# yechuan51/huffman

Hardware: AMD Instinct MI355X
Metric: encode + decode throughput GB/s and % HBM3E peak, 16 GiB Zipf(1.1), 1/2/4/8 GPU (higher is better)
Workload: dtype u8; 1 GPU; 16 GiB Zipf(1.1) bytes per GPU: hist16 -> codebook -> pack -> decode, one global bit stream; bytes_per_gpu=17179869184, total_bytes=17179869184, symbols_per_gpu=8589934592, parallelism=single, payload_bytes_rank0=12416072164, max_code_len=22

## Files before the change

### huffman_amd/csrc/hz_kernels.hip

```cpp
#include <stdio.h>
#include <stdlib.h>

#include <type_traits>

#include "hz_device.h"

namespace hz {

struct DecArgs {
    const uint32_t* words;
    uint64_t nwords;
    uint32_t bit_adj;
    uint64_t nsym;
    uint64_t nblocks;
    const unsigned long long* starts;
    const unsigned long long* subs;
    uint64_t start0;
    const uint32_t* lds_img;
    uint32_t lds_words;
    uint32_t region_words;
    int k;
    int min_len;
    int max_len;
    int level_bits;
// ... 362 lines not shown
                }
                x = make_uint4(q[0], q[1], q[2], q[3]);
            }
            if (DESC)
                reinterpret_cast<uint4*>(stg)[npc_max - 1 - p] = make_uint4(bswap32(x.w), bswap32(x.z), bswap32(x.y), bswap32(x.x));
            else
                reinterpret_cast<uint4*>(stg)[p] = make_uint4(bswap32(x.x), bswap32(x.y), bswap32(x.z), bswap32(x.w));
        }
    }
    for (uint32_t p = (uint32_t)lane + kStageUnroll * kWave; p < npc; p += kWave) {
        const uint4 x = dec_stage_load(a, w0 + 4ull * p);
        if (DESC)
            reinterpret_cast<uint4*>(stg)[npc_max - 1 - p] = make_uint4(bswap32(x.w), bswap32(x.z), bswap32(x.y), bswap32(x.x));
        else
            reinterpret_cast<uint4*>(stg)[p] = make_uint4(bswap32(x.x), bswap32(x.y), bswap32(x.z), bswap32(x.w));
    }
}

constexpr int kPfStep = 4;
template <typename A>
HZ_DEV void dec_wave_pipe(const A& a, const uint32_t* lds, uint32_t* stg, uint32_t slot, uint64_t b,
                          uint64_t stride, int lane) {
    const uint32_t* l2g = a.l2;
    constexpr int C = kChainsPerLane;
    static_assert(C == 4, "two halves of two chains");
    PipeMeta mc, mn, mn2;
    uint4 sc[kStageUnroll], sn[kStageUnroll];
    dec_meta_load(a, b, lane, mc);
    dec_meta_load(a, b + stride, lane, mn);
    dec_stage_prefetch(a, mc, lane, sc);
    for (; b < a.nblocks; b += stride) {
        uint64_t w0;
        dec_stage_commit(a, mc, slot >> 2, stg, lane, sc, w0);
        uint32_t off[C];
        dec_chain_offsets(mc.sub, mc.b0, mc.b1 - mc.b0, lane, off);
        const uint32_t base = (uint32_t)(mc.b0 + a.bit_adj - (w0 << 5));
        uint32_t pos[C];
#pragma unroll
        for (int c = 0; c < C; ++c) pos[c] = base + off[c];
        __builtin_amdgcn_wave_barrier();
        uint32_t pk[kSPT / 2];
        PipeLane st[C];
        uint32_t g[C];
        auto finish = [&](int c, int q) {
            const uint32_t ee = (st[c].e >> 31) ? st[c].e : g[c];
            pos[c] += lut_leaf_len(ee);
            const uint32_t sym = lut_leaf_sym(ee);
            const int i = (c * kChainSyms + q) >> 1;
            if (q & 1) pk[i] |= sym << 16;
            else pk[i] = sym;
        };
        auto issue2 = [&](int c) {
            dec_pipe_lds2(a, lds, stg, pos[c], pos[c + 1], st[c], st[c + 1]);
            g[c] = l2g[st[c].gi];
            g[c + 1] = l2g[st[c + 1].gi];
        };
        issue2(0);
#pragma unroll
        for (int q = 0; q < kChainSyms; ++q) {
            issue2(2);
            if (q == kPfStep) {
                dec_stage_prefetch(a, mn, lane, sn);
                dec_meta_load(a, b + 2 * stride, lane, mn2);
            }
            finish(0, q);
            finish(1, q);
            if (q + 1 < kChainSyms) issue2(0);
            finish(2, q);
            finish(3, q);
        }
        __builtin_amdgcn_wave_barrier();
        dec_store(a, b, lane, pk);
        mc = mn;
        mn = mn2;
#pragma unroll
        for (int u = 0; u < kStageUnroll; ++u) sc[u] = sn[u];
    }
}

template <typename A>
HZ_DEV void dec_wave_pipe2(const A& a, const uint32_t* lds, uint32_t* stg, uint32_t slot, uint64_t b,
                           uint64_t stride, int lane) {
    constexpr int C = 2 * kChainsPerLane;
    static_assert(kChainsPerLane == 4, "four pairs of chains over two blocks");
    const __amdgpu_buffer_rsrc_t l2r = lut_l2_rsrc(a.l2);
    [[maybe_unused]] const uint32_t stg_bit = (uint32_t)(stg - lds) * 32u - 1u;
    PipeMeta mc[2], mn[2], mn2[2];
    uint4 sc[2][kStageUnroll], sn[2][kStageUnroll];
#pragma unroll
    for (int j = 0; j < 2; ++j) {
        dec_meta_load(a, b + j, lane, mc[j]);
        dec_meta_load(a, b + stride + j, lane, mn[j]);
    }
#pragma unroll
    for (int j = 0; j < 2; ++j) dec_stage_prefetch(a, mc[j], lane, sc[j]);
    for (; b < a.nblocks; b += stride) {
        uint32_t p1[C];
#pragma unroll
        for (int j = 0; j < 2; ++j) {
            uint64_t w0;
            dec_stage_commit<true>(a, mc[j], slot >> 2, stg + j * slot, lane, sc[j], w0);
            uint32_t off[kChainsPerLane];
            dec_chain_offsets(mc[j].sub, mc[j].b0, mc[j].b1 - mc[j].b0, lane, off);
            const uint32_t top = (uint32_t)(stg - lds) + (uint32_t)(j + 1) * slot - 1u;
            const uint32_t base = top * 32u - (uint32_t)(mc[j].b0 + a.bit_adj - (w0 << 5));
#pragma unroll
            for (int c = 0; c < kChainsPerLane; ++c) p1[j * kChainsPerLane + c] = base - off[c];
        }
        __builtin_amdgcn_wave_barrier();
        uint32_t pk[2][kSPT / 2];
        PipeLane st[C];
        uint32_t g[C];
        auto finish = [&](int c, int q) {
            const uint32_t ee = st[c].e > g[c] ? st[c].e : g[c];
            p1[c] -= ee >> 24;
            const int i = ((c % kChainsPerLane) * kChainSyms + q) >> 1;
            if (q & 1) pk[c / kChainsPerLane][i] = __builtin_amdgcn_perm(ee, pk[c / kChainsPerLane][i], 0x06050201u);
            else pk[c / kChainsPerLane][i] = ee;
        };
        auto issue4 = [&](int c, int q) {
            __builtin_amdgcn_s_setprio(2);
            dec_pipe_ldsn<4>(a, lds, p1 + c, st + c, 16u * (uint32_t)q);
#pragma unroll
            for (int t = 0; t < 4; ++t)
                g[c + t] = __builtin_amdgcn_raw_buffer_load_b32(l2r, st[c + t].gi, 0, 0);
            __builtin_amdgcn_s_setprio(0);
        };
        issue4(0, 0);
#pragma unroll
        for (int q = 0; q < kChainSyms; ++q) {
            issue4(4, q);
            if (q == kPfStep) {
#pragma unroll
                for (int j = 0; j < 2; ++j) dec_stage_prefetch(a, mn[j], lane, sn[j]);
#pragma unroll
                for (int j = 0; j < 2; ++j) dec_meta_load(a, b + 2 * stride + j, lane, mn2[j]);
            }
#pragma unroll
            for (int c = 0; c < 4; ++c) finish(c, q);
            if (q + 1 < kChainSyms) issue4(0, q + 1);
#pragma unroll
            for (int c = 4; c < 8; ++c) finish(c, q);
        }
        __builtin_amdgcn_wave_barrier();
#pragma unroll
        for (int j = 0; j < 2; ++j)
            if (b + j < a.nblocks) dec_store(a, b + j, lane, pk[j]);
#pragma unroll
        for (int j = 0; j < 2; ++j) {
            mc[j] = mn[j];
            mn[j] = mn2[j];
#pragma unroll
            for (int u = 0; u < kStageUnroll; ++u) sc[j][u] = sn[j][u];
        }
    }
}

constexpr int kDecPipe2Threads = 512;
template <int MODE, bool WIDE, int PIPE>
__global__ __launch_bounds__(PIPE == 2 ? kDecPipe2Threads : 1024) void k_decode(DecArgs a) {
    extern __shared__ __attribute__((aligned(16))) uint32_t lds[];
    copy_lds_table(lds, a.lds_img, a.lds_words);
    const int lane = threadIdx.x & 63;
    const uint32_t wid = wave_id();
    const uint32_t slot = (uint32_t)__builtin_amdgcn_readfirstlane((int)dec_slot_words(a.starts[a.nblocks + 1], a.max_len));
    const uint32_t nwave = blockDim.x >> 6;
    if constexpr (PIPE == 2) {
        uint32_t nw2 = a.region_words / (2 * slot);
        nw2 = nw2 < nwave ? nw2 : nwave;
        if (nw2 > 0) {
            if (wid >= nw2) return;
            const uint64_t b = 2 * ((uint64_t)blockIdx.x * nw2 + wid), stride = 2 * (uint64_t)gridDim.x * nw2;
            dec_wave_pipe2(a, lds, lds + a.lds_words + wid * 2 * slot, slot, b, stride, lane);
            return;
        }
    }
    uint32_t nw = a.region_words / slot;
    nw = nw < nwave ? nw : nwave;
    if (wid >= nw) return;
    uint32_t* stg = lds + a.lds_words + wid * slot;
    const uint64_t b = (uint64_t)blockIdx.x * nw + wid, stride = (uint64_t)gridDim.x * nw;
    if constexpr (PIPE != 0) {
        dec_wave_pipe(a, lds, stg, slot, b, stride, lane);
    } else {
        for (uint64_t bb = b; bb < a.nblocks; bb += stride) dec_group<MODE, WIDE, 1>(a, lds, stg, slot, bb, lane);
    }
}

HZ_DEV void fixed16_step(const uint16_t* t16, const uint32_t (&ww)[5], uint32_t pos, uint32_t (&o)[4]) {
    const uint32_t sh = pos & 31;
#pragma unroll
    for (int t = 0; t < 4; ++t) {
        const uint32_t cw = sh ? __builtin_amdgcn_alignbit(ww[t], ww[t + 1], 32u - sh) : ww[t];
        o[t] = (uint32_t)t16[cw >> 16] | ((uint32_t)t16[cw & 0xffffu] << 16);
    }
}

__global__ __launch_bounds__(1024) void k_decode_fixed16_blk(DecArgs a, uint64_t nb) {
    extern __shared__ __attribute__((aligned(16))) uint32_t lds[];
    copy_lds_table(lds, a.lds_img, a.lds_words);
    const uint16_t* t16 = reinterpret_cast<const uint16_t*>(lds);
    const uint64_t p0 = (a.starts ? a.starts[0] : a.start0) + a.bit_adj;
    const uint32_t* w = a.words + (p0 >> 5);
    const u32x4a4* w4 = reinterpret_cast<const u32x4a4*>(w);
    uint4* o4 = reinterpret_cast<uint4*>(a.out);
    const int lane = threadIdx.x & 63;
    const uint64_t W = (uint64_t)gridDim.x * (blockDim.x >> 6);
    uint64_t b = (uint64_t)blockIdx.x * (blockDim.x >> 6) + (threadIdx.x >> 6);
    constexpr uint32_t kBW = kBlockSyms / 2;
    auto load = [&](uint64_t bb, u32x4a4 (&x)[kChainsPerLane], uint32_t& nw) {
        bb = bb < nb ? bb : 0;
#pragma unroll
        for (int c = 0; c < kChainsPerLane; ++c) x[c] = w4[bb * (kBW / 4) + c * kWave + lane];
        nw = w[(bb + 1) * kBW];
    };
    u32x4a4 nx[kChainsPerLane];
    uint32_t nn = 0;
    if (b < nb) load(b, nx, nn);
    for (; b < nb; b += W) {
        u32x4a4 x[kChainsPerLane];
#pragma unroll
        for (int c = 0; c < kChainsPerLane; ++c) x[c] = nx[c];
        const uint32_t after = nn;
        load(b + W, nx, nn);
#pragma unroll
        for (int c = 0; c < kChainsPerLane; ++c) {
            uint32_t nxt = (uint32_t)__builtin_amdgcn_update_dpp(0, (int)x[c].x, kDppWaveShl1, 0xf, 0xf, false);
            const uint32_t first_next = c + 1 < kChainsPerLane ? readlane(x[c + 1 < kChainsPerLane ? c + 1 : c].x, 0) : after;
            if (lane == 63) nxt = first_next;
            const uint32_t ww[5] = {bswap32(x[c].x), bswap32(x[c].y), bswap32(x[c].z), bswap32(x[c].w), bswap32(nxt)};
            uint32_t o[4];
            fixed16_step(t16, ww, (uint32_t)p0, o);
            store_nt16(o4 + b * (kBlockSyms / 8) + c * kWave + lane, make_uint4(o[0], o[1], o[2], o[3]));
        }
    }
}

// ... 2228 lines not shown
```

### huffman_amd/csrc/hz_pack.hip

```cpp
#include <mutex>
#include <set>
#include <utility>

#include "hz_device.h"

namespace hz {

hipError_t ensure_lds_limit(const void* fn, int bytes) {
    int dev = 0;
    hipError_t e = hipGetDevice(&dev);
    if (e != hipSuccess) return e;
    static std::mutex mu;
    static std::set<std::pair<std::pair<const void*, int>, int>> done;
    std::lock_guard<std::mutex> lk(mu);
    const auto key = std::make_pair(std::make_pair(fn, dev), bytes);
    if (done.count(key)) return hipSuccess;
    if ((e = hipFuncSetAttribute(fn, hipFuncAttributeMaxDynamicSharedMemorySize, bytes)) != hipSuccess) return e;
    done.insert(key);
    return hipSuccess;
}

struct PackArgs {
    const uint8_t* in;
    uint64_t nsym;
    uint64_t nblocks;
    const uint32_t* lds_img;
    uint32_t lds_words;
    const unsigned long long* wide;
    const uint32_t* esc;
    const uint32_t* len8_img;
    uint32_t hot_mask;
    uint32_t hw_mask;
    uint32_t* out;
    uint64_t out_words;
    uint32_t lead;
    unsigned long long* blk;
    const unsigned long long* blk_start;
    unsigned long long* index;
    unsigned long long* index_sub;
    uint32_t* err;
    uint32_t slot_words;
    const unsigned long long* rstart;
    uint64_t bpr, nranges;
    unsigned long long* cold;
};

template <int MODE> struct PackEnt { using T = uint32_t; static constexpr int kShift = 26; };
template <> struct PackEnt<ENC_WIDE> { using T = uint64_t; static constexpr int kShift = 56; };
template <int MODE>
HZ_DEV uint32_t ent_len(typename PackEnt<MODE>::T e) {
    if constexpr (MODE == ENC_WIDE) return (uint32_t)(e >> 56);
    else return __builtin_amdgcn_ubfe((uint32_t)e, 26, 5);
}

template <typename T, int SH>
HZ_DEV T pack_dense_one(const uint32_t* lds, uint32_t s) {
    const uint32_t bit = s * 17u;
    const uint32_t w = bit >> 5;
    const uint64_t two = ((uint64_t)lds[w + 1] << 32) | lds[w];
    const uint32_t f = (uint32_t)(two >> (bit & 31)) & 0x1ffffu;
    const uint32_t L = f ? 16u - (uint32_t)__builtin_ctz(f) : 0u;
    return f ? (T)((L << SH) | (f >> (17u - L))) : (T)0;
}

struct PackIn {
    uint32_t raw[kSPT / 2];
    uint32_t psym;
    uint64_t bstart;
};

HZ_DEV void pack_prefetch(const PackArgs& a, uint64_t blk, int lane, PackIn& x) {
    const uint64_t sym0 = blk * kBlockSyms + (uint64_t)lane * kSPT;
    const uint64_t ls = sym0 + kSPT <= a.nsym ? sym0 : 0;
    const uint4* p = reinterpret_cast<const uint4*>(a.in + 2 * ls);
#pragma unroll
    for (int q = 0; q < kSPT / 8; ++q) {
        const uint4 v = p[q];
        x.raw[4 * q] = v.x; x.raw[4 * q + 1] = v.y; x.raw[4 * q + 2] = v.z; x.raw[4 * q + 3] = v.w;
    }
    const uint64_t ps = blk ? blk * kBlockSyms - 32 + (uint64_t)(lane & 31) : 0;
    x.psym = *reinterpret_cast<const uint16_t*>(a.in + 2 * ps);
    x.bstart = a.blk_start ? a.blk_start[blk] : 0;
}

struct HotLook {
    uint32_t x[kSPT], mk[kSPT], v[kSPT];
    uint32_t xx, xmk, xv;
};
template <bool FULL>
HZ_DEV void hot_issue(const PackArgs& a, const uint32_t (&raw)[kSPT / 2], uint32_t xs, HotLook& h, int nvalid = kSPT) {
    const uint32_t m2 = a.hot_mask | (a.hot_mask << 16);
    uint32_t ad[kSPT];
#pragma unroll
    for (int j = 0; j < kSPT / 2; ++j) {
        const uint32_t r = raw[j];
        const uint32_t sgn = __builtin_bit_cast(uint32_t, __builtin_bit_cast(hz_i16x2, r) >> (hz_i16x2){15, 15});
        const uint32_t sl = r ^ (sgn & m2);
        const uint32_t hi8 = __builtin_bit_cast(uint32_t, __builtin_bit_cast(hz_u16x2, sl) >> (hz_u16x2){8, 8});
        uint32_t hw, a0, a1;
        asm("v_bitop3_b32 %0, %1, %2, %3 bitop3:0x6c" : "=v"(hw) : "s"(a.hw_mask), "v"(sl), "v"(hi8));
        asm("v_lshlrev_b32_sdwa %0, %1, %2 dst_sel:DWORD dst_unused:UNUSED_PAD src0_sel:DWORD src1_sel:WORD_0"
            : "=v"(a0) : "v"(2u), "v"(hw));
        asm("v_lshlrev_b32_sdwa %0, %1, %2 dst_sel:DWORD dst_unused:UNUSED_PAD src0_sel:DWORD src1_sel:WORD_1"
            : "=v"(a1) : "v"(2u), "v"(hw));
        ad[2 * j] = a0;
        ad[2 * j + 1] = a1;
    }
#pragma unroll
    for (int k = 0; k < kSPT; ++k) {
        h.x[k] = lds_at(ad[k]);
        if (!FULL) h.x[k] = k < nvalid ? h.x[k] : 0u;
    }
    uint32_t xslot = xs ^ ((uint32_t)((int32_t)(xs << 16) >> 31) & a.hot_mask);
    xslot = hot_word(xslot & 0x7fffu) << 2;
    h.xx = lds_at(xslot);
    const char* esc = reinterpret_cast<const char*>(a.esc);
#pragma unroll
    for (int k = 0; k < kSPT; ++k) {
        const uint32_t tag = (k & 1) ? raw[k >> 1] : raw[k >> 1] << 16;
        h.mk[k] = (uint32_t)((int32_t)(h.x[k] ^ tag) >> 31);
        h.v[k] = *reinterpret_cast<const uint32_t*>(esc + (ad[k] & h.mk[k]));
    }
    h.xmk = (uint32_t)((int32_t)(h.xx ^ (xs << 16)) >> 31);
    h.xv = *reinterpret_cast<const uint32_t*>(esc + (xslot & h.xmk));
}
HZ_DEV void hot_finish(const HotLook& h, uint32_t (&e)[kSPT], uint32_t& xe) {
#pragma unroll
    for (int k = 0; k < kSPT; ++k) {
        uint32_t r;
        asm volatile("v_bfi_b32 %0, %1, %2, %3" : "=v"(r) : "v"(h.mk[k]), "v"(h.v[k]), "v"(h.x[k]));
        e[k] = r;
    }
    uint32_t r;
    asm volatile("v_bfi_b32 %0, %1, %2, %3" : "=v"(r) : "v"(h.xmk), "v"(h.xv), "v"(h.xx));
    xe = r;
}

struct NoMid {
    HZ_DEV void operator()() const {}
};
template <int MODE, bool FULL, typename Mid = NoMid>
HZ_DEV void pack_lookup(const PackArgs& a, const uint32_t* lds, uint64_t sym0, int nvalid, uint32_t (&raw)[kSPT / 2],
                        typename PackEnt<MODE>::T (&e)[kSPT], uint32_t xs, typename PackEnt<MODE>::T& xe,
                        Mid mid = Mid()) {
    using T = typename PackEnt<MODE>::T;
    constexpr int SH = PackEnt<MODE>::kShift;
    if (!FULL) {
#pragma unroll
        for (int k = 0; k < kSPT / 2; ++k) {
            uint32_t w = 0;
            if (2 * k < nvalid) w = (uint32_t)a.in[2 * (sym0 + 2 * k)] | ((uint32_t)a.in[2 * (sym0 + 2 * k) + 1] << 8);
            if (2 * k + 1 < nvalid)
                w |= ((uint32_t)a.in[2 * (sym0 + 2 * k + 1)] | ((uint32_t)a.in[2 * (sym0 + 2 * k + 1) + 1] << 8)) << 16;
            raw[k] = w;
        }
    }
    if constexpr (MODE == ENC_DENSE) {
#pragma unroll
        for (int k = 0; k < kSPT; ++k) {
            const uint32_t s = (raw[k >> 1] >> (16 * (k & 1))) & 0xffffu;
            const uint32_t bit = s * 17u;
            const uint32_t w = bit >> 5;
            const uint64_t two = ((uint64_t)lds[w + 1] << 32) | lds[w];
            const uint32_t f = (uint32_t)(two >> (bit & 31)) & 0x1ffffu;
            const uint32_t L = f ? 16u - (uint32_t)__builtin_ctz(f) : 0u;
            e[k] = ((FULL || k < nvalid) && f) ? (T)((L << SH) | (f >> (17u - L))) : (T)0;
        }
        xe = pack_dense_one<T, SH>(lds, xs);
        mid();
    } else if constexpr (MODE == ENC_HOT) {
        HotLook h;
        hot_issue<FULL>(a, raw, xs, h, nvalid);
        mid();
        hot_finish(h, e, xe);
    } else {
#pragma unroll
        for (int k = 0; k < kSPT; ++k) {
            const uint32_t s = (raw[k >> 1] >> (16 * (k & 1))) & 0xffffu;
            e[k] = (FULL || k < nvalid) ? (T)a.wide[s] : (T)0;
        }
        xe = (T)a.wide[xs];
        mid();
    }
}

constexpr int kCountThreads = 1024;
constexpr int kCountUnroll = 2;

__global__ __launch_bounds__(kCountThreads) void k_pack_count(PackArgs a) {
    extern __shared__ __attribute__((aligned(16))) uint32_t lds[];
    {
        const uint4* src = reinterpret_cast<const uint4*>(a.len8_img);
        uint4* dst = reinterpret_cast<uint4*>(lds);
        for (uint32_t i = threadIdx.x; i < kLen8LdsBytes / 16; i += blockDim.x) dst[i] = src[i];
        __syncthreads();
    }
    const uint8_t* l8 = reinterpret_cast<const uint8_t*>(lds);
    const int lane = threadIdx.x & 63;
    const uint64_t W = (uint64_t)gridDim.x * (blockDim.x >> 6);
    const uint64_t full = a.nsym / kBlockSyms;
    uint64_t blk = (uint64_t)blockIdx.x * (blockDim.x >> 6) + (threadIdx.x >> 6);
    for (; blk + (kCountUnroll - 1) * W < full; blk += kCountUnroll * W) {
        uint4 v[kCountUnroll][kSPT / 8];
#pragma unroll
        for (int u = 0; u < kCountUnroll; ++u) {
            const uint4* p = reinterpret_cast<const uint4*>(a.in + 2 * (blk + u * W) * kBlockSyms) + lane;
#pragma unroll
            for (int q = 0; q < kSPT / 8; ++q) v[u][q] = p[q * kWave];
        }
#pragma unroll
        for (int u = 0; u < kCountUnroll; ++u) {
            uint32_t n = 0;
#pragma unroll
            for (int q = 0; q < kSPT / 8; ++q) {
                const uint32_t wd[4] = {v[u][q].x, v[u][q].y, v[u][q].z, v[u][q].w};
#pragma unroll
                for (int k = 0; k < 8; ++k) n += l8[len8_index((wd[k >> 1] >> (16 * (k & 1))) & 0xffffu)];
            }
// ... 68 lines not shown
    }
}

constexpr int kPackMaxWaves = 8;
constexpr double kPackSlotMargin = 1.12;
constexpr int kPackWriteThreads = 64 * kPackMaxWaves;
constexpr int kPackCopyIters = 16;

template <int MODE>
struct PackBlk {
    typename PackEnt<MODE>::T e[kSPT];
    typename PackEnt<MODE>::T pe;
    uint32_t n, ex_n, bits;
    uint32_t nc[kChainsPerLane];
    int nvalid;
};

template <int MODE, bool FULL_ONLY = false, typename Mid = NoMid>
HZ_DEV void pack_block_lookup(const PackArgs& a, const uint32_t* lds, uint64_t blk, int lane, PackIn& in,
                              PackBlk<MODE>& b, Mid mid = Mid()) {
    const uint64_t sym0 = blk * kBlockSyms + (uint64_t)lane * kSPT;
    if constexpr (FULL_ONLY) {
        b.nvalid = kSPT;
        pack_lookup<MODE, true>(a, lds, sym0, b.nvalid, in.raw, b.e, in.psym, b.pe, mid);
        return;
    }
    b.nvalid = sym0 >= a.nsym ? 0 : (a.nsym - sym0 >= (uint64_t)kSPT ? kSPT : (int)(a.nsym - sym0));
    if (__ballot(b.nvalid != kSPT) == 0)
        pack_lookup<MODE, true>(a, lds, sym0, b.nvalid, in.raw, b.e, in.psym, b.pe, mid);
    else
        pack_lookup<MODE, false>(a, lds, sym0, b.nvalid, in.raw, b.e, in.psym, b.pe, mid);
}

struct PackOut {
    bool pending, fits;
    uint64_t base4, blk, bstart, sub;
    uint32_t sh4, nwords;
};

HZ_DEV void pack_copyout(const PackArgs& a, const uint32_t* slot, int lane, const PackOut& p) {
    if (!p.pending) return;
    if (p.fits) {
        const uint32_t sh4 = p.sh4;
        const uint32_t wend = sh4 + p.nwords;
        const uint32_t cf = sh4 ? 1u : 0u, cl = wend >> 2;
        const uint32_t nhead = sh4 ? 4u - sh4 : 0u, ntail = wend & 3u;
        {
            const uint32_t i = (uint32_t)lane < nhead ? sh4 + (uint32_t)lane : sh4;
            a.out[p.base4 + i] = bswap32(slot[i]);
        }
#pragma unroll
        for (int it = 0; it < kPackCopyIters / 4; ++it) {
            uint32_t c = cf + (uint32_t)lane + (uint32_t)it * kWave;
            c = c < cl ? c : cl - 1;
            const uint4 v = reinterpret_cast<const uint4*>(slot)[c];
            reinterpret_cast<uint4*>(a.out + p.base4)[c] = make_uint4(bswap32(v.x), bswap32(v.y), bswap32(v.z), bswap32(v.w));
        }
        {
            const uint32_t i = (uint32_t)lane < ntail ? 4u * cl + (uint32_t)lane : sh4;
            a.out[p.base4 + i] = bswap32(slot[i]);
        }
    }
    if (a.index) {
        a.index_sub[p.blk * kWave + lane] = p.sub;
        if (lane == 0) a.index[p.blk] = p.bstart;
    }
    __builtin_amdgcn_wave_barrier();
}

template <int MODE>
HZ_DEV void pack_block_count(int lane, PackBlk<MODE>& b) {
    uint32_t n = 0;
#pragma unroll
    for (int k = 0; k < kSPT; ++k) {
        if (k % kChainSyms == 0) b.nc[k / kChainSyms] = n;
        n += ent_len<MODE>(b.e[k]);
    }
    const uint32_t sn = wave_incl_sum(n);
    b.n = n;
    b.ex_n = sn - n;
    b.bits = readlane(sn, 63);
}

template <int MODE, bool SLOT_ONLY = false>
HZ_DEV void pack_block_emit(const PackArgs& a, uint32_t* slot, uint64_t blk, int lane, const PackBlk<MODE>& b,
                            uint64_t bstart, uint64_t& max_bits, PackOut* defer = nullptr) {
    using T = typename PackEnt<MODE>::T;
    constexpr int SH = PackEnt<MODE>::kShift;
    constexpr T CMASK = (T(1) << SH) - 1;
    const uint64_t sym0 = blk * kBlockSyms + (uint64_t)lane * kSPT;
    const uint32_t n = b.n, ex_n = b.ex_n;
    const uint64_t bend = bstart + b.bits;
    uint32_t ptail = a.lead;
    if (blk > 0) {
        uint32_t pn = ent_len<MODE>(b.pe);
        uint32_t pt = (uint32_t)(b.pe & CMASK);
        auto step = [&](uint32_t on, uint32_t ot) {
            pt = pn >= 32 ? pt : ((ot << pn) | pt);
            pn += on;
        };
        step(dpp0<kDppRowShr1>(pn), dpp0<kDppRowShr1>(pt));
        step(dpp0<kDppRowShr2>(pn), dpp0<kDppRowShr2>(pt));
        step(dpp0<kDppRowShr4>(pn), dpp0<kDppRowShr4>(pt));
        step(dpp0<kDppRowShr8>(pn), dpp0<kDppRowShr8>(pt));
        step(dpp0<kDppRowBcast15, 0xa>(pn), dpp0<kDppRowBcast15, 0xa>(pt));
        ptail = readlane(pt, 31);
    }
    const uint64_t o = bstart + ex_n;
    const bool fits = ((bend + 31) >> 5) <= a.out_words;
    if (!fits && lane == 0) atomicOr(a.err, 4u);
    const bool last = blk + 1 == a.nblocks;
    const uint64_t wfirst = bstart >> 5;
    const uint32_t nwords = (uint32_t)((bend >> 5) - wfirst);
    const uint32_t sh4 = (uint32_t)(wfirst & 3);
    if (SLOT_ONLY || (slot && !last && nwords + sh4 <= a.slot_words)) {
        uint32_t* sl = slot + sh4;
        uint64_t acc = 0;
        if constexpr (MODE == ENC_WIDE) {
            uint32_t na = (uint32_t)(o & 31);
            pack_emit<MODE, true>(b.e, acc, na, sl + (uint32_t)((o >> 5) - wfirst), true);
        } else {
            pack_emit_lds<MODE>(b.e, acc, (uint32_t)(o - (wfirst << 5)), sl);
        }
        const uint32_t prev = (uint32_t)__builtin_amdgcn_update_dpp((int)ptail, (int)(uint32_t)acc, kDppWaveShr1,
                                                                    0xf, 0xf, false);
        const uint32_t h = (uint32_t)(o & 31);
        if (h) sl[(uint32_t)((o >> 5) - wfirst)] |= prev << (32 - h);
        __builtin_amdgcn_wave_barrier();
        if (MODE != ENC_WIDE && defer) {
            defer->pending = true;
            defer->fits = fits;
            defer->base4 = wfirst & ~3ull;
            defer->sh4 = sh4;
            defer->nwords = nwords;
            defer->blk = blk;
            defer->bstart = bstart;
            uint64_t sub = 0;
#pragma unroll
            for (int c = 0; c < kChainsPerLane; ++c)
                sub |= (uint64_t)(((uint32_t)bstart + ex_n + b.nc[c]) & 0xffffu) << (16 * c);
            defer->sub = sub;
            max_bits = b.bits > max_bits ? b.bits : max_bits;
            return;
        }
        if (fits) {
            if constexpr (MODE != ENC_WIDE) {
                const uint64_t base4 = wfirst & ~3ull;
                const uint32_t wend = sh4 + nwords;
                const uint32_t cf = sh4 ? 1u : 0u, cl = wend >> 2;
                const uint32_t nhead = sh4 ? 4u - sh4 : 0u, ntail = wend & 3u;
                {
                    const uint32_t i = (uint32_t)lane < nhead ? sh4 + (uint32_t)lane : sh4;
                    a.out[base4 + i] = bswap32(slot[i]);
                }
#pragma unroll
                for (int it = 0; it < kPackCopyIters / 4; ++it) {
                    uint32_t c = cf + (uint32_t)lane + (uint32_t)it * kWave;
                    c = c < cl ? c : cl - 1;
                    const uint4 v = reinterpret_cast<const uint4*>(slot)[c];
                    reinterpret_cast<uint4*>(a.out + base4)[c] =
                        make_uint4(bswap32(v.x), bswap32(v.y), bswap32(v.z), bswap32(v.w));
                }
                {
                    const uint32_t i = (uint32_t)lane < ntail ? 4u * cl + (uint32_t)lane : sh4;
                    a.out[base4 + i] = bswap32(slot[i]);
                }
            } else {
                for (uint32_t w = lane; w < nwords; w += kWave) a.out[wfirst + w] = bswap32(sl[w]);
            }
        }
        __builtin_amdgcn_wave_barrier();
    } else if constexpr (!SLOT_ONLY) {
        uint64_t t64 = 0;
#pragma unroll
        for (int k = 0; k < kSPT; ++k) {
            const uint32_t L = ent_len<MODE>(b.e[k]);
            t64 = L ? ((t64 << L) | (uint64_t)(b.e[k] & CMASK)) : t64;
        }
        uint32_t tn = n, st = (uint32_t)t64;
#pragma unroll
        for (int d = 1; d < 64; d <<= 1) {
            const uint32_t on = shfl_up_u32(tn, d), ot = shfl_up_u32(st, d);
            if (lane >= d) {
                st = tn >= 32 ? st : (tn == 0 ? ot : ((ot << tn) | st));
                tn += on;
            }
        }
        uint32_t ex_t = shfl_up_u32(st, 1);
        if (lane == 0) ex_t = 0;
        const uint32_t pre = ex_n >= 32 ? ex_t : (ex_n == 0 ? ptail : ((ptail << ex_n) | ex_t));
        uint32_t na = (uint32_t)(o & 31);
        uint64_t acc = na ? (uint64_t)(pre & ((1u << na) - 1u)) : 0ull;
        uint32_t* dst = a.out + (o >> 5);
        pack_emit<MODE, false>(b.e, acc, na, dst, fits);
        dst += (uint32_t)(((o & 31) + n) >> 5);
        if (fits && b.nvalid > 0 && sym0 + (uint64_t)b.nvalid == a.nsym && na > 0)
            *dst = bswap32((uint32_t)(acc << (32 - na)));
    }
    if (a.index) {
        uint64_t sub = 0;
#pragma unroll
        for (int c = 0; c < kChainsPerLane; ++c)
            sub |= (uint64_t)(((uint32_t)bstart + ex_n + b.nc[c]) & 0xffffu) << (16 * c);
        a.index_sub[blk * kWave + lane] = sub;
        if (lane == 0) {
            a.index[blk] = bstart;
            if (last) a.index[a.nblocks] = bend;
        }
        max_bits = bend - bstart > max_bits ? bend - bstart : max_bits;
    }
}


template <int MODE, bool RNG, bool SPLIT>
__global__ __launch_bounds__(kPackWriteThreads) void k_pack_write(PackArgs a) {
    extern __shared__ __attribute__((aligned(16))) uint32_t lds[];
    if constexpr (MODE != ENC_WIDE) copy_lds_table(lds, a.lds_img, a.lds_words);
    const int lane = threadIdx.x & 63;
    constexpr bool kSplit = SPLIT && MODE != ENC_WIDE;
    uint32_t* slot = a.slot_words ? lds + a.lds_words + (threadIdx.x >> 6) * a.slot_words : nullptr;
    const uint64_t W = (uint64_t)gridDim.x * (blockDim.x >> 6);
    const uint64_t gw = (uint64_t)blockIdx.x * (blockDim.x >> 6) + (threadIdx.x >> 6);
    uint64_t max_bits = 0;
    uint64_t blk = gw, r = gw, rend = 0, run = 0;
    if (RNG) {
        blk = r < a.nranges ? r * a.bpr : a.nblocks;
        rend = blk + a.bpr < a.nblocks ? blk + a.bpr : a.nblocks;
        run = r < a.nranges ? a.rstart[r] : 0;
    }
    PackOut po;
    po.pending = false;
    if constexpr (MODE == ENC_HOT && kSplit) {
        auto next = [&](uint64_t b, bool& newr, uint64_t& nrun) -> uint64_t {
            newr = false;
            nrun = 0;
            if (!RNG) return b + W;
            if (b + 1 < rend) return b + 1;
            r += W;
            newr = true;
            const uint64_t n = r < a.nranges ? r * a.bpr : a.nblocks;
            rend = n + a.bpr < a.nblocks ? n + a.bpr : a.nblocks;
            nrun = r < a.nranges ? a.rstart[r] : 0;
            return n;
        };
        bool nb_newr;
        uint64_t nb_run;
        uint64_t nb = next(blk, nb_newr, nb_run);
        PackIn nx;
        HotLook hl;
        uint64_t bst_cur = run;
        if (blk < a.nblocks) {
            PackIn cur;
            pack_prefetch(a, blk, lane, cur);
            hot_issue<true>(a, cur.raw, cur.psym, hl);
            if (!RNG) bst_cur = cur.bstart;
            pack_prefetch(a, nb < a.nblocks ? nb : blk, lane, nx);
        }
        while (blk < a.nblocks) {
            bool nn_newr;
            uint64_t nn_run;
            const uint64_t nnb = next(nb, nn_newr, nn_run);
            PackBlk<MODE> b;
            hot_finish(hl, b.e, b.pe);
            b.nvalid = kSPT;
            __builtin_amdgcn_s_setprio(2);
            hot_issue<true>(a, nx.raw, nx.psym, hl);
            __builtin_amdgcn_s_setprio(0);
            const uint64_t nbst = nx.bstart;
            pack_copyout(a, slot, lane, po);
            po.pending = false;
            const uint64_t pb = nnb < a.nblocks ? nnb : (nb < a.nblocks ? nb : blk);
            pack_prefetch(a, pb, lane, nx);
            pack_block_count<MODE>(lane, b);
            const uint64_t bst = bst_cur;
            const uint64_t wfirst = bst >> 5;
            const uint32_t nwords = (uint32_t)(((bst + b.bits) >> 5) - wfirst), sh4 = (uint32_t)(wfirst & 3);
            if (blk + 1 == a.nblocks || nwords + sh4 > a.slot_words) {
                if (lane == 0) {
                    const unsigned long long i = atomicAdd(a.cold, 1ull);
                    a.cold[1 + 2 * i] = blk;
                    a.cold[2 + 2 * i] = bst;
                }
            } else {
                pack_block_emit<MODE, true>(a, slot, blk, lane, b, bst, max_bits, &po);
            }
            if (RNG) run = nb_newr ? nb_run : run + b.bits;
            bst_cur = RNG ? run : nbst;
            blk = nb;
            nb = nnb;
            nb_newr = nn_newr;
            nb_run = nn_run;
        }
        pack_copyout(a, slot, lane, po);
        if (a.index && lane == 0 && max_bits) atomicMax(a.index + a.nblocks + 1, (unsigned long long)max_bits);
        return;
    }
    PackIn nx;
    if (blk < a.nblocks) pack_prefetch(a, blk, lane, nx);
    while (blk < a.nblocks) {
        uint64_t nb = blk + W, nrun = 0;
        bool newr = false;
        if (RNG) {
            if (blk + 1 < rend) {
                nb = blk + 1;
            } else {
                r += W;
                newr = true;
                nb = r < a.nranges ? r * a.bpr : a.nblocks;
                rend = nb + a.bpr < a.nblocks ? nb + a.bpr : a.nblocks;
                nrun = r < a.nranges ? a.rstart[r] : 0;
            }
        }
        PackIn cur = nx;
        PackBlk<MODE> b;
        pack_block_lookup<MODE, kSplit>(a, lds, blk, lane, cur, b, [&]() { pack_copyout(a, slot, lane, po); });
        po.pending = false;
        pack_prefetch(a, nb < a.nblocks ? nb : blk, lane, nx);
        pack_block_count<MODE>(lane, b);
        const uint64_t bst = RNG ? run : cur.bstart;
        if constexpr (kSplit) {
            const uint64_t wfirst = bst >> 5;
            const uint32_t nwords = (uint32_t)(((bst + b.bits) >> 5) - wfirst), sh4 = (uint32_t)(wfirst & 3);
            if (blk + 1 == a.nblocks || nwords + sh4 > a.slot_words) {
                if (lane == 0) {
                    const unsigned long long i = atomicAdd(a.cold, 1ull);
                    a.cold[1 + 2 * i] = blk;
                    a.cold[2 + 2 * i] = bst;
                }
            } else {
                pack_block_emit<MODE, true>(a, slot, blk, lane, b, bst, max_bits, &po);
            }
        } else {
            pack_block_emit<MODE>(a, slot, blk, lane, b, bst, max_bits, &po);
        }
        if (RNG) run = newr ? nrun : run + b.bits;
        blk = nb;
    }
    pack_copyout(a, slot, lane, po);
    if (a.index && lane == 0 && max_bits) atomicMax(a.index + a.nblocks + 1, (unsigned long long)max_bits);
}

template <int MODE>
__global__ __launch_bounds__(kPackWriteThreads) void k_pack_cold(PackArgs a) {
    extern __shared__ __attribute__((aligned(16))) uint32_t lds[];
    const uint64_t n = a.cold[0];
    const uint64_t waves = blockDim.x >> 6, W = (uint64_t)gridDim.x * waves;
    if ((uint64_t)blockIdx.x * waves >= n) return;
    if constexpr (MODE != ENC_WIDE) copy_lds_table(lds, a.lds_img, a.lds_words);
    const int lane = threadIdx.x & 63;
    uint64_t max_bits = 0;
    for (uint64_t i = (uint64_t)blockIdx.x * waves + (threadIdx.x >> 6); i < n; i += W) {
        const uint64_t blk = a.cold[1 + 2 * i], bst = a.cold[2 + 2 * i];
        PackIn in;
        pack_prefetch(a, blk, lane, in);
        PackBlk<MODE> b;
        pack_block_lookup<MODE>(a, lds, blk, lane, in, b);
        pack_block_count<MODE>(lane, b);
        pack_block_emit<MODE>(a, nullptr, blk, lane, b, bst, max_bits, nullptr);
    }
    if (a.index && lane == 0 && max_bits) atomicMax(a.index + a.nblocks + 1, (unsigned long long)max_bits);
}

__global__ __launch_bounds__(kPackThreads) void k_pack_fixed16_blk(PackArgs a, uint64_t start_bit, uint64_t nb) {
    extern __shared__ __attribute__((aligned(16))) uint32_t lds[];
    copy_lds_table(lds, a.lds_img, a.lds_words);
    const uint16_t* c16 = reinterpret_cast<const uint16_t*>(lds);
    const uint32_t sb = (uint32_t)(start_bit & 31);
    const int lane = threadIdx.x & 63;
// ... 400 lines not shown
```

Measured before the change: 811.1 GB/s.

## Stagger decode block pairs across half-steps and carry pack tails between blocks

The two-block decode pipeline is rebuilt so the two blocks run half a chain out of phase. Each block's store, stage commit and next prefetch now happen mid-loop, overlapping the other block's lookups. This is meant to remove the wave-wide bubble at the end of each iteration, at the cost of a single staging buffer and more complex control flow. In the ranged hot pack path, the previous block's 32-bit tail is carried in a register from the last emitted accumulator instead of re-reading the preceding 32 symbols and running a DPP scan. It falls back to a recompute when a range starts.

```diff
diff --git a/huffman_amd/csrc/hz_kernels.hip b/huffman_amd/csrc/hz_kernels.hip
--- a/huffman_amd/csrc/hz_kernels.hip
+++ b/huffman_amd/csrc/hz_kernels.hip
@@ -468,77 +468,93 @@
 HZ_DEV void dec_wave_pipe2(const A& a, const uint32_t* lds, uint32_t* stg, uint32_t slot, uint64_t b,
                            uint64_t stride, int lane) {
     constexpr int C = 2 * kChainsPerLane;
+    constexpr int H = kChainSyms / 2;
     static_assert(kChainsPerLane == 4, "four pairs of chains over two blocks");
+    static_assert(kChainSyms == 8 && kPfStep == H, "a block's prefetch issues at the top of its second half");
     const __amdgpu_buffer_rsrc_t l2r = lut_l2_rsrc(a.l2);
-    [[maybe_unused]] const uint32_t stg_bit = (uint32_t)(stg - lds) * 32u - 1u;
-    PipeMeta mc[2], mn[2], mn2[2];
-    uint4 sc[2][kStageUnroll], sn[2][kStageUnroll];
-#pragma unroll
-    for (int j = 0; j < 2; ++j) {
-        dec_meta_load(a, b + j, lane, mc[j]);
-        dec_meta_load(a, b + stride + j, lane, mn[j]);
-    }
-#pragma unroll
-    for (int j = 0; j < 2; ++j) dec_stage_prefetch(a, mc[j], lane, sc[j]);
+    PipeMeta mn[2], mn2;
+    uint4 sn[kStageUnroll];
+    uint32_t p1[C];
+    uint32_t pk[2][kSPT / 2];
+    PipeLane st[C];
+    uint32_t g[C];
+    auto commit = [&](int j) {
+        uint64_t w0;
+        dec_stage_commit<true>(a, mn[j], slot >> 2, stg + j * slot, lane, sn, w0);
+        uint32_t off[kChainsPerLane];
+        dec_chain_offsets(mn[j].sub, mn[j].b0, mn[j].b1 - mn[j].b0, lane, off);
+        const uint32_t top = (uint32_t)(stg - lds) + (uint32_t)(j + 1) * slot - 1u;
+        const uint32_t base = top * 32u - (uint32_t)(mn[j].b0 + a.bit_adj - (w0 << 5));
+#pragma unroll
+        for (int c = 0; c < kChainsPerLane; ++c) p1[j * kChainsPerLane + c] = base - off[c];
+        mn[j] = mn2;
+    };
+    auto prefetch = [&](int j, uint64_t after) {
+        dec_stage_prefetch(a, mn[j], lane, sn);
+        dec_meta_load(a, after, lane, mn2);
+    };
+    auto finish = [&](int c, int q) {
+        const uint32_t ee = st[c].e > g[c] ? st[c].e : g[c];
+        p1[c] -= ee >> 24;
+        const int i = ((c % kChainsPerLane) * kChainSyms + q) >> 1;
+        if (q & 1) pk[c / kChainsPerLane][i] = __builtin_amdgcn_perm(ee, pk[c / kChainsPerLane][i], 0x06050201u);
+        else pk[c / kChainsPerLane][i] = ee;
+    };
+    auto issue4 = [&](int c, int q) {
+        __builtin_amdgcn_s_setprio(2);
+        dec_pipe_ldsn<4>(a, lds, p1 + c, st + c, 16u * (uint32_t)q);
+#pragma unroll
+        for (int t = 0; t < 4; ++t)
+            g[c + t] = __builtin_amdgcn_raw_buffer_load_b32(l2r, st[c + t].gi, 0, 0);
+        __builtin_amdgcn_s_setprio(0);
+    };
+    auto finish4 = [&](int c, int q) {
+#pragma unroll
+        for (int t = 0; t < 4; ++t) finish(c + t, q);
+    };
+    if (b >= a.nblocks) return;
+    dec_meta_load(a, b, lane, mn[0]);
+    dec_meta_load(a, b + 1, lane, mn[1]);
+    prefetch(0, b + stride);
+    commit(0);
+    prefetch(1, b + 1 + stride);
+    commit(1);
+    __builtin_amdgcn_wave_barrier();
+    issue4(0, 0);
+#pragma unroll
+    for (int q = 0; q < H; ++q) {
+        finish4(0, q);
+        issue4(0, q + 1);
+    }
     for (; b < a.nblocks; b += stride) {
-        uint32_t p1[C];
-#pragma unroll
-        for (int j = 0; j < 2; ++j) {
-            uint64_t w0;
-            dec_stage_commit<true>(a, mc[j], slot >> 2, stg + j * slot, lane, sc[j], w0);
-            uint32_t off[kChainsPerLane];
-            dec_chain_offsets(mc[j].sub, mc[j].b0, mc[j].b1 - mc[j].b0, lane, off);
-            const uint32_t top = (uint32_t)(stg - lds) + (uint32_t)(j + 1) * slot - 1u;
-            const uint32_t base = top * 32u - (uint32_t)(mc[j].b0 + a.bit_adj - (w0 << 5));
-#pragma unroll
-            for (int c = 0; c < kChainsPerLane; ++c) p1[j * kChainsPerLane + c] = base - off[c];
+#pragma unroll
+        for (int t = 0; t < H; ++t) {
+            issue4(4, t);
+            if (t == 0) prefetch(0, b + 2 * stride);
+            finish4(0, H + t);
+            if (t + 1 < H) {
+                issue4(0, H + t + 1);
+            } else {
+                __builtin_amdgcn_wave_barrier();
+                dec_store(a, b, lane, pk[0]);
+                commit(0);
+                __builtin_amdgcn_wave_barrier();
+                issue4(0, 0);
+            }
+            finish4(4, t);
+        }
+#pragma unroll
+        for (int t = 0; t < H; ++t) {
+            issue4(4, H + t);
+            if (t == 0) prefetch(1, b + 1 + 2 * stride);
+            finish4(0, t);
+            issue4(0, t + 1);
+            finish4(4, H + t);
         }
         __builtin_amdgcn_wave_barrier();
-        uint32_t pk[2][kSPT / 2];
-        PipeLane st[C];
-        uint32_t g[C];
-        auto finish = [&](int c, int q) {
-            const uint32_t ee = st[c].e > g[c] ? st[c].e : g[c];
-            p1[c] -= ee >> 24;
-            const int i = ((c % kChainsPerLane) * kChainSyms + q) >> 1;
-            if (q & 1) pk[c / kChainsPerLane][i] = __builtin_amdgcn_perm(ee, pk[c / kChainsPerLane][i], 0x06050201u);
-            else pk[c / kChainsPerLane][i] = ee;
-        };
-        auto issue4 = [&](int c, int q) {
-            __builtin_amdgcn_s_setprio(2);
-            dec_pipe_ldsn<4>(a, lds, p1 + c, st + c, 16u * (uint32_t)q);
-#pragma unroll
-            for (int t = 0; t < 4; ++t)
-                g[c + t] = __builtin_amdgcn_raw_buffer_load_b32(l2r, st[c + t].gi, 0, 0);
-            __builtin_amdgcn_s_setprio(0);
-        };
-        issue4(0, 0);
-#pragma unroll
-        for (int q = 0; q < kChainSyms; ++q) {
-            issue4(4, q);
-            if (q == kPfStep) {
-#pragma unroll
-                for (int j = 0; j < 2; ++j) dec_stage_prefetch(a, mn[j], lane, sn[j]);
-#pragma unroll
-                for (int j = 0; j < 2; ++j) dec_meta_load(a, b + 2 * stride + j, lane, mn2[j]);
-            }
-#pragma unroll
-            for (int c = 0; c < 4; ++c) finish(c, q);
-            if (q + 1 < kChainSyms) issue4(0, q + 1);
-#pragma unroll
-            for (int c = 4; c < 8; ++c) finish(c, q);
-        }
+        if (b + 1 < a.nblocks) dec_store(a, b + 1, lane, pk[1]);
+        commit(1);
         __builtin_amdgcn_wave_barrier();
-#pragma unroll
-        for (int j = 0; j < 2; ++j)
-            if (b + j < a.nblocks) dec_store(a, b + j, lane, pk[j]);
-#pragma unroll
-        for (int j = 0; j < 2; ++j) {
-            mc[j] = mn[j];
-            mn[j] = mn2[j];
-#pragma unroll
-            for (int u = 0; u < kStageUnroll; ++u) sc[j][u] = sn[j][u];
-        }
     }
 }
 
diff --git a/huffman_amd/csrc/hz_pack.hip b/huffman_amd/csrc/hz_pack.hip
--- a/huffman_amd/csrc/hz_pack.hip
+++ b/huffman_amd/csrc/hz_pack.hip
@@ -69,6 +69,7 @@
     uint64_t bstart;
 };
 
+template <bool PSYM = true>
 HZ_DEV void pack_prefetch(const PackArgs& a, uint64_t blk, int lane, PackIn& x) {
     const uint64_t sym0 = blk * kBlockSyms + (uint64_t)lane * kSPT;
     const uint64_t ls = sym0 + kSPT <= a.nsym ? sym0 : 0;
@@ -78,8 +79,11 @@
         const uint4 v = p[q];
         x.raw[4 * q] = v.x; x.raw[4 * q + 1] = v.y; x.raw[4 * q + 2] = v.z; x.raw[4 * q + 3] = v.w;
     }
-    const uint64_t ps = blk ? blk * kBlockSyms - 32 + (uint64_t)(lane & 31) : 0;
-    x.psym = *reinterpret_cast<const uint16_t*>(a.in + 2 * ps);
+    x.psym = 0;
+    if constexpr (PSYM) {
+        const uint64_t ps = blk ? blk * kBlockSyms - 32 + (uint64_t)(lane & 31) : 0;
+        x.psym = *reinterpret_cast<const uint16_t*>(a.in + 2 * ps);
+    }
     x.bstart = a.blk_start ? a.blk_start[blk] : 0;
 }
 
@@ -87,7 +91,7 @@
     uint32_t x[kSPT], mk[kSPT], v[kSPT];
     uint32_t xx, xmk, xv;
 };
-template <bool FULL>
+template <bool FULL, bool XS = true>
 HZ_DEV void hot_issue(const PackArgs& a, const uint32_t (&raw)[kSPT / 2], uint32_t xs, HotLook& h, int nvalid = kSPT) {
     const uint32_t m2 = a.hot_mask | (a.hot_mask << 16);
     uint32_t ad[kSPT];
@@ -113,7 +117,7 @@
     }
     uint32_t xslot = xs ^ ((uint32_t)((int32_t)(xs << 16) >> 31) & a.hot_mask);
     xslot = hot_word(xslot & 0x7fffu) << 2;
-    h.xx = lds_at(xslot);
+    if constexpr (XS) h.xx = lds_at(xslot);
     const char* esc = reinterpret_cast<const char*>(a.esc);
 #pragma unroll
     for (int k = 0; k < kSPT; ++k) {
@@ -121,9 +125,12 @@
         h.mk[k] = (uint32_t)((int32_t)(h.x[k] ^ tag) >> 31);
         h.v[k] = *reinterpret_cast<const uint32_t*>(esc + (ad[k] & h.mk[k]));
     }
-    h.xmk = (uint32_t)((int32_t)(h.xx ^ (xs << 16)) >> 31);
-    h.xv = *reinterpret_cast<const uint32_t*>(esc + (xslot & h.xmk));
-}
+    if constexpr (XS) {
+        h.xmk = (uint32_t)((int32_t)(h.xx ^ (xs << 16)) >> 31);
+        h.xv = *reinterpret_cast<const uint32_t*>(esc + (xslot & h.xmk));
+    }
+}
+template <bool XS = true>
 HZ_DEV void hot_finish(const HotLook& h, uint32_t (&e)[kSPT], uint32_t& xe) {
 #pragma unroll
     for (int k = 0; k < kSPT; ++k) {
@@ -131,9 +138,11 @@
         asm volatile("v_bfi_b32 %0, %1, %2, %3" : "=v"(r) : "v"(h.mk[k]), "v"(h.v[k]), "v"(h.x[k]));
         e[k] = r;
     }
-    uint32_t r;
-    asm volatile("v_bfi_b32 %0, %1, %2, %3" : "=v"(r) : "v"(h.xmk), "v"(h.xv), "v"(h.xx));
-    xe = r;
+    if constexpr (XS) {
+        uint32_t r;
+        asm volatile("v_bfi_b32 %0, %1, %2, %3" : "=v"(r) : "v"(h.xmk), "v"(h.xv), "v"(h.xx));
+        xe = r;
+    }
 }
 
 struct NoMid {
@@ -368,9 +377,48 @@
     b.bits = readlane(sn, 63);
 }
 
-template <int MODE, bool SLOT_ONLY = false>
+template <int MODE>
+HZ_DEV uint32_t pack_tail_scan(typename PackEnt<MODE>::T pe) {
+    using T = typename PackEnt<MODE>::T;
+    constexpr T CMASK = (T(1) << PackEnt<MODE>::kShift) - 1;
+    uint32_t pn = ent_len<MODE>(pe);
+    uint32_t pt = (uint32_t)(pe & CMASK);
+    auto step = [&](uint32_t on, uint32_t ot) {
+        pt = pn >= 32 ? pt : ((ot << pn) | pt);
+        pn += on;
+    };
+    step(dpp0<kDppRowShr1>(pn), dpp0<kDppRowShr1>(pt));
+    step(dpp0<kDppRowShr2>(pn), dpp0<kDppRowShr2>(pt));
+    step(dpp0<kDppRowShr4>(pn), dpp0<kDppRowShr4>(pt));
+    step(dpp0<kDppRowShr8>(pn), dpp0<kDppRowShr8>(pt));
+    step(dpp0<kDppRowBcast15, 0xa>(pn), dpp0<kDppRowBcast15, 0xa>(pt));
+    return readlane(pt, 31);
+}
+
+HZ_DEV uint32_t hot_prev_tail(const PackArgs& a, uint64_t blk, int lane) {
+    if (blk == 0) return a.lead;
+    const uint32_t xs = *reinterpret_cast<const uint16_t*>(a.in + 2 * (blk * kBlockSyms - 32 + (uint64_t)(lane & 31)));
+    uint32_t xslot = xs ^ ((uint32_t)((int32_t)(xs << 16) >> 31) & a.hot_mask);
+    xslot = hot_word(xslot & 0x7fffu) << 2;
+    const uint32_t xx = lds_at(xslot);
+    const uint32_t xmk = (uint32_t)((int32_t)(xx ^ (xs << 16)) >> 31);
+    const uint32_t xv = *reinterpret_cast<const uint32_t*>(reinterpret_cast<const char*>(a.esc) + (xslot & xmk));
+    return pack_tail_scan<ENC_HOT>((xv & xmk) | (xx & ~xmk));
+}
+
+template <int MODE>
+HZ_DEV uint32_t pack_own_tail(const PackBlk<MODE>& b) {
+    static_assert(MODE != ENC_WIDE, "u32 entries");
+    uint32_t t = 0;
+#pragma unroll
+    for (int k = 0; k < kSPT; ++k) t = (t << ent_len<MODE>(b.e[k])) | (b.e[k] & ((1u << PackEnt<MODE>::kShift) - 1u));
+    return readlane(t, 63);
+}
+
+template <int MODE, bool SLOT_ONLY = false, bool CARRY = false>
 HZ_DEV void pack_block_emit(const PackArgs& a, uint32_t* slot, uint64_t blk, int lane, const PackBlk<MODE>& b,
-                            uint64_t bstart, uint64_t& max_bits, PackOut* defer = nullptr) {
+                            uint64_t bstart, uint64_t& max_bits, PackOut* defer = nullptr, uint32_t* tail = nullptr) {
+    static_assert(!CARRY || (SLOT_ONLY && MODE != ENC_WIDE), "the carried tail is the slot path's");
     using T = typename PackEnt<MODE>::T;
     constexpr int SH = PackEnt<MODE>::kShift;
     constexpr T CMASK = (T(1) << SH) - 1;
@@ -378,20 +426,8 @@
     const uint32_t n = b.n, ex_n = b.ex_n;
     const uint64_t bend = bstart + b.bits;
     uint32_t ptail = a.lead;
-    if (blk > 0) {
-        uint32_t pn = ent_len<MODE>(b.pe);
-        uint32_t pt = (uint32_t)(b.pe & CMASK);
-        auto step = [&](uint32_t on, uint32_t ot) {
-            pt = pn >= 32 ? pt : ((ot << pn) | pt);
-            pn += on;
-        };
-        step(dpp0<kDppRowShr1>(pn), dpp0<kDppRowShr1>(pt));
-        step(dpp0<kDppRowShr2>(pn), dpp0<kDppRowShr2>(pt));
-        step(dpp0<kDppRowShr4>(pn), dpp0<kDppRowShr4>(pt));
-        step(dpp0<kDppRowShr8>(pn), dpp0<kDppRowShr8>(pt));
-        step(dpp0<kDppRowBcast15, 0xa>(pn), dpp0<kDppRowBcast15, 0xa>(pt));
-        ptail = readlane(pt, 31);
-    }
+    if constexpr (CARRY) ptail = *tail;
+    else if (blk > 0) ptail = pack_tail_scan<MODE>(b.pe);
     const uint64_t o = bstart + ex_n;
     const bool fits = ((bend + 31) >> 5) <= a.out_words;
     if (!fits && lane == 0) atomicOr(a.err, 4u);
@@ -410,6 +446,7 @@
         }
         const uint32_t prev = (uint32_t)__builtin_amdgcn_update_dpp((int)ptail, (int)(uint32_t)acc, kDppWaveShr1,
                                                                     0xf, 0xf, false);
+        if constexpr (CARRY) *tail = readlane((uint32_t)acc, 63);
         const uint32_t h = (uint32_t)(o & 31);
         if (h) sl[(uint32_t)((o >> 5) - wfirst)] |= prev << (32 - h);
         __builtin_amdgcn_wave_barrier();
@@ -529,6 +566,9 @@
             nrun = r < a.nranges ? a.rstart[r] : 0;
             return n;
         };
+        constexpr bool kCarry = RNG;
+        uint32_t tail = 0;
+        bool have_tail = false;
         bool nb_newr;
         uint64_t nb_run;
         uint64_t nb = next(blk, nb_newr, nb_run);
@@ -537,26 +577,26 @@
         uint64_t bst_cur = run;
         if (blk < a.nblocks) {
             PackIn cur;
-            pack_prefetch(a, blk, lane, cur);
-            hot_issue<true>(a, cur.raw, cur.psym, hl);
+            pack_prefetch<!kCarry>(a, blk, lane, cur);
+            hot_issue<true, !kCarry>(a, cur.raw, cur.psym, hl);
             if (!RNG) bst_cur = cur.bstart;
-            pack_prefetch(a, nb < a.nblocks ? nb : blk, lane, nx);
+            pack_prefetch<!kCarry>(a, nb < a.nblocks ? nb : blk, lane, nx);
         }
         while (blk < a.nblocks) {
             bool nn_newr;
             uint64_t nn_run;
             const uint64_t nnb = next(nb, nn_newr, nn_run);
             PackBlk<MODE> b;
-            hot_finish(hl, b.e, b.pe);
+            hot_finish<!kCarry>(hl, b.e, b.pe);
             b.nvalid = kSPT;
             __builtin_amdgcn_s_setprio(2);
-            hot_issue<true>(a, nx.raw, nx.psym, hl);
+            hot_issue<true, !kCarry>(a, nx.raw, nx.psym, hl);
             __builtin_amdgcn_s_setprio(0);
             const uint64_t nbst = nx.bstart;
             pack_copyout(a, slot, lane, po);
             po.pending = false;
             const uint64_t pb = nnb < a.nblocks ? nnb : (nb < a.nblocks ? nb : blk);
-            pack_prefetch(a, pb, lane, nx);
+            pack_prefetch<!kCarry>(a, pb, lane, nx);
             pack_block_count<MODE>(lane, b);
             const uint64_t bst = bst_cur;
             const uint64_t wfirst = bst >> 5;
@@ -567,9 +607,14 @@
                     a.cold[1 + 2 * i] = blk;
                     a.cold[2 + 2 * i] = bst;
                 }
+                if constexpr (kCarry) tail = pack_own_tail<MODE>(b);
+            } else if constexpr (kCarry) {
+                if (!have_tail) tail = hot_prev_tail(a, blk, lane);
+                pack_block_emit<MODE, true, true>(a, slot, blk, lane, b, bst, max_bits, &po, &tail);
             } else {
                 pack_block_emit<MODE, true>(a, slot, blk, lane, b, bst, max_bits, &po);
             }
+            have_tail = !nb_newr;
             if (RNG) run = nb_newr ? nb_run : run + b.bits;
             bst_cur = RNG ? run : nbst;
             blk = nb;
```

Result: faster. 835.3 GB/s, median of 6 (+3.0%).
